# alphacep/vosk-tts

Measured on AMD Instinct MI355X. Metric: audio_samples_per_sec, higher is better.
Workload: dtype f32

## Files before the change

vosk_tts_amd/csrc/engine_model.hip.h:

```cpp
#pragma once
struct ConvW {
  float* w = nullptr;
  float* w16 = nullptr;
  float* wb = nullptr;
  float* bias = nullptr;
  int M = 0, Mpad = 0, Cin = 0, K = 0, n_sg = 0;
};
struct EncLayerW {
  ConvW qkv, o, f1, f2;
  float *ek = nullptr, *ev = nullptr, *g1 = nullptr, *b1 = nullptr, *g2 = nullptr, *b2 = nullptr;
};
struct EncoderW {
  std::vector<EncLayerW> layers;
  int H = 0, F = 0, K = 0;
  int nh = 0, W = 0;
};
struct DDSW {
  std::vector<float*> sw, sb, g1, b1, g2, b2;
  std::vector<float*> swk[3];
  std::vector<float*> wt;
  std::vector<ConvW> pw;
};
struct ConvFlowW {
  float *pre_w = nullptr, *pre_b = nullptr;
  DDSW dds;
  ConvW proj;
};
struct CouplingW {
  ConvW pre, post;
  EncoderW enc;
  std::vector<ConvW> in_layers, rs_layers;
  std::vector<ConvW> rsx;
  ConvW skip_post;
  int cond_off = 0;
};
struct MonoW {
  EncoderW enc;
  float *post_w = nullptr, *post_b = nullptr;
};
struct ResBlockW {
  ConvW c1[VITS_MAX_RESD], c2[VITS_MAX_RESD];
  int K = 0;
  int dil[VITS_MAX_RESD] = {0};
};
struct UpW {
  ConvW w;
  int u = 0, Ku = 0, cout = 0, taps = 0, pad_l = 0, halo = 0;
  int shift[8] = {0};
};
struct DecNeeds {
  int pre_out = 0, post_out = 0, tail_cols = 0;
  int ups_q[VITS_MAX_UPS] = {0};
  int c1_out[VITS_MAX_UPS][VITS_MAX_RESD] = {{0}}, c2_out[VITS_MAX_UPS][VITS_MAX_RESD] = {{0}};
};
struct DecGeom {
  struct Stage {
    int cin = 0, cout = 0;
    int u = 0, taps = 0;
    int rate_in = 1, rate_out = 1;
  } st[VITS_MAX_UPS];
  int n_ups = 0;
  int post_rows = 1, post_pad = 3;
  bool reflect = false;
  bool has_mb = false;
  int final_rate = 1;
  long long samples_per_frame = 1;
  DecNeeds needs;
  int rag_halo = 32;
};
static DecGeom dec_geom(const vits_hparams& hp) {
  DecGeom G;
  const bool istft = hp.dec_type == 0 || hp.dec_type == 2 || hp.dec_type == 3, filt = hp.dec_type == 0 || hp.dec_type == 2;
  G.n_ups = hp.n_ups;
  double rf = 3.0;
  double span = 0;
  for (int j = 0; j < hp.n_resk; ++j) {
    double sp = 0;
    for (int d = 0; d < hp.n_resd; ++d) sp += (hp.res_kernels[j] - 1) * hp.res_dilations[j][d] / 2.0 + (hp.res_kernels[j] - 1) / 2.0;
    if (sp > span) span = sp;
  }
  long long rate = 1;
  int C = hp.dec_initial_channel;
  for (int i = 0; i < hp.n_ups; ++i) {
    DecGeom::Stage& S = G.st[i];
    S.u = hp.up_rates[i]; S.taps = (hp.up_kernels[i] + S.u - 1) / S.u;
    S.cin = C; S.cout = C / 2;
    S.rate_in = (int)rate;
    rf += (double)(S.taps / 2 + 1) / (double)rate;
    rate *= S.u;
    S.rate_out = (int)rate;
    rf += span / (double)rate;
    C = S.cout;
  }
  G.final_rate = (int)rate;
  G.samples_per_frame = istft ? rate * hp.istft_hop * hp.subbands : rate;
  G.reflect = istft; G.post_pad = istft ? 4 : 3;
  G.post_rows = istft ? hp.subbands * (hp.istft_n_fft + 2) : 1;
  G.has_mb = filt;
  rf += 4.0 / (double)rate;
  if (filt) rf += ((double)hp.istft_n_fft / hp.istft_hop + (hp.pqmf_taps / 2.0) / hp.subbands / hp.istft_hop) / (double)rate;
  if (hp.dec_type == 3) rf += ((double)hp.istft_n_fft / hp.istft_hop) / (double)rate;
  G.rag_halo = std::max((int)ceil(rf) + 2, 32);

  DecNeeds& N = G.needs;
  int need = 0;
  if (istft) need = (hp.istft_n_fft + hp.istft_hop - 1) / hp.istft_hop + 2;
  if (filt) need += ((hp.pqmf_taps / 2 + hp.subbands - 1) / hp.subbands + hp.istft_hop - 1) / hp.istft_hop;
  N.tail_cols = need;
  N.post_out = need + 1;
  need += 4;
  for (int i = hp.n_ups - 1; i >= 0; --i) {
    for (int d = hp.n_resd - 1; d >= 0; --d) {
      int h2 = 0, h1 = 0;
      for (int j = 0; j < hp.n_resk; ++j) {
        const int k = hp.res_kernels[j];
        h2 = std::max(h2, (k - 1) / 2);
// ... 69 lines not shown

static const float* tget(vits_model* m, int ndim, int d0, int d1, int d2, const char* fmt, ...) {
  char name[160];
  va_list ap;
  va_start(ap, fmt);
  vsnprintf(name, sizeof name, fmt, ap);
  va_end(ap);
  for (uint32_t i = 0; i < m->n_entries; ++i) {
    const vits_blob_entry* e = &m->entries[i];
    if (strncmp(e->name, name, sizeof e->name) == 0) {
      const int want[3] = {d0, d1, d2};
      if ((int)e->ndim != ndim) { m->missing = true; fail(VITS_ERR_BLOB, "tensor %s: ndim %u != %d", name, e->ndim, ndim); return nullptr; }
      for (int k = 0; k < ndim && k < 3; ++k)
        if (want[k] >= 0 && (int)e->dims[k] != want[k]) {
          m->missing = true;
          fail(VITS_ERR_BLOB, "tensor %s: dim %d is %u, expected %d", name, k, e->dims[k], want[k]);
          return nullptr;
        }
      return reinterpret_cast<const float*>(m->blob + e->offset);
    }
  }
  m->missing = true;
  fail(VITS_ERR_BLOB, "tensor %s missing from blob", name);
  return nullptr;
}

static bool thas(const vits_model* m, const char* name) {
  for (uint32_t i = 0; i < m->n_entries; ++i)
    if (strncmp(m->entries[i].name, name, sizeof m->entries[i].name) == 0) return true;
  return false;
}

static size_t align_up(size_t v, size_t a) { return (v + a - 1) / a * a; }

static void* weight_alloc(vits_model* m, size_t bytes) {
  bytes = align_up(bytes ? bytes : 4, 256);
  constexpr size_t guard = (size_t)64 << 10;
  if (m->slab_used + bytes + guard > m->slab_bytes) {
    size_t want = m->blob_bytes + m->blob_bytes / 4 + ((size_t)8 << 20);
    if (!m->allocs.empty()) want = (size_t)32 << 20;
    if (want < bytes + guard) want = bytes + guard;
    want = align_up(want, (size_t)2 << 20);
    void* d = nullptr;
    if (hipMalloc(&d, want) != hipSuccess) return nullptr;
    m->allocs.push_back(d);
    m->slab = static_cast<char*>(d);
    m->slab_bytes = want;
    m->slab_used = 0;
  }
  void* p = m->slab + m->slab_used;
  m->slab_used += bytes;
  return p;
}

static float* upload(vits_model* m, const float* host, size_t n) {
  if (!host) return nullptr;
  void* d = weight_alloc(m, n * sizeof(float));
  if (!d) { m->missing = true; fail(VITS_ERR_NOMEM, "hipMalloc of %zu floats failed", n); return nullptr; }
  if (hipMemcpy(d, host, n * sizeof(float), hipMemcpyHostToDevice) != hipSuccess) { m->missing = true; fail(VITS_ERR_DEVICE, "hipMemcpy H2D failed"); return nullptr; }
  return static_cast<float*>(d);
}

template <typename F, typename F16>
static ConvW make_conv2(vits_model* m, int M, int Cin, int K, const float* bias, F src, bool small16, F16 src16) {
  ConvW c;
  c.M = M; c.Mpad = cdiv(M, 32) * 32; c.Cin = Cin; c.K = K;
  if (Cin % CONV_CI_T != 0) { m->missing = true; fail(VITS_ERR_UNSUPPORTED, "conv C_in=%d is not a multiple of %d", Cin, CONV_CI_T); return c; }
  c.n_sg = Cin / CONV_CI_T * 2 * K;
  std::vector<float> packed((size_t)c.Mpad * Cin * K);
  pack_conv_weights(packed.data(), c.Mpad, Cin, K, [&](int row, int ci, int kk) -> float { return row < M ? src(row, ci, kk) : 0.f; });
  c.w = upload(m, packed.data(), packed.size());
  if (small16) {
    const int Mp16 = cdiv(M, 16) * 16;
    packed.assign((size_t)Mp16 * Cin * K, 0.f);
    pack_conv_weights16(packed.data(), Mp16, Cin, K, [&](int row, int ci, int kk) -> float { return row < M ? src16(row, ci, kk) : 0.f; });
    c.w16 = upload(m, packed.data(), packed.size());
  }
  c.bias = bias ? upload(m, bias, M) : nullptr;
  return c;
}
template <typename F>
static ConvW make_conv(vits_model* m, int M, int Cin, int K, const float* bias, F src, bool small16 = true) {
  return make_conv2(m, M, Cin, K, bias, src, small16, src);
}

template <typename F>
static void add_bf3_packing(vits_model* m, ConvW& c, F src) {
  if (!c.w || c.Mpad % 32 || c.Cin % CONV_CI_T) return;
  std::vector<uint16_t> pk((size_t)c.Mpad * c.Cin * c.K * 2 + 2 * 128 * 8, 0);
  const int M = c.M;
  pack_conv_weights_bf3(pk.data(), c.Mpad, c.Cin, c.K, [&](int row, int ci, int kk) -> float { return row < M ? src(row, ci, kk) : 0.f; });
  c.wb = upload(m, reinterpret_cast<const float*>(pk.data()), pk.size() / 2);
}
static ConvW conv_from(vits_model* m, const char* name, int Cout, int Cin, int K, bool has_bias, bool small16 = true, bool bf3 = false) {
  const float* w = tget(m, 3, Cout, Cin, K, "%s.weight", name);
  const float* b = has_bias ? tget(m, 1, Cout, -1, -1, "%s.bias", name) : nullptr;
  if (m->missing) return ConvW();
  auto src = [&](int r, int ci, int kk) { return w[((size_t)r * Cin + ci) * K + kk]; };
  ConvW c = make_conv(m, Cout, Cin, K, b, src, small16);
  if (bf3) add_bf3_packing(m, c, src);
  return c;
}

static void load_encoder(vits_model* m, EncoderW& E, const char* pfx, int n_layers, int H, int F, int K, int nh, int W) {
  const vits_hparams& hp = m->hp;
  const int dk = H / nh, NW = 2 * W + 1;
  E.H = H; E.F = F; E.K = K; E.nh = nh; E.W = W;
  E.layers.resize(n_layers);
  char nm[200];
  for (int i = 0; i < n_layers && !m->missing; ++i) {
    EncLayerW& L = E.layers[i];
    const float* wq = tget(m, 3, H, H, 1, "%s.attn_layers.%d.conv_q.weight", pfx, i);
    const float* wk = tget(m, 3, H, H, 1, "%s.attn_layers.%d.conv_k.weight", pfx, i);
    const float* wv = tget(m, 3, H, H, 1, "%s.attn_layers.%d.conv_v.weight", pfx, i);
    const float* bq = tget(m, 1, H, -1, -1, "%s.attn_layers.%d.conv_q.bias", pfx, i);
    const float* bk = tget(m, 1, H, -1, -1, "%s.attn_layers.%d.conv_k.bias", pfx, i);
    const float* bv = tget(m, 1, H, -1, -1, "%s.attn_layers.%d.conv_v.bias", pfx, i);
    if (m->missing) return;
    std::vector<float> b3(3 * H);
    memcpy(b3.data(), bq, sizeof(float) * H); memcpy(b3.data() + H, bk, sizeof(float) * H); memcpy(b3.data() + 2 * H, bv, sizeof(float) * H);
    auto qkv_src = [&](int r, int ci, int) {
      const float* w = r < H ? wq : (r < 2 * H ? wk : wv);
      return w[(size_t)(r % H) * H + ci];
    };
    L.qkv = make_conv(m, 3 * H, H, 1, b3.data(), qkv_src);
    const bool bf3 = hp.conv_precision == 1 && H % 64 == 0 && F % 64 == 0;
    if (bf3) add_bf3_packing(m, L.qkv, qkv_src);
    snprintf(nm, sizeof nm, "%s.attn_layers.%d.conv_o", pfx, i);
    L.o = conv_from(m, nm, H, H, 1, true, true, bf3);
    if (W >= 0) {
      L.ek = upload(m, tget(m, 3, 1, NW, dk, "%s.attn_layers.%d.emb_rel_k", pfx, i), (size_t)NW * dk);
      L.ev = upload(m, tget(m, 3, 1, NW, dk, "%s.attn_layers.%d.emb_rel_v", pfx, i), (size_t)NW * dk);
    }
    snprintf(nm, sizeof nm, "%s.ffn_layers.%d.conv_1", pfx, i);
    L.f1 = conv_from(m, nm, F, H, K, true, true, bf3);
    snprintf(nm, sizeof nm, "%s.ffn_layers.%d.conv_2", pfx, i);
    L.f2 = conv_from(m, nm, H, F, K, true, true, bf3);
    L.g1 = upload(m, tget(m, 1, H, -1, -1, "%s.norm_layers_1.%d.gamma", pfx, i), H);
    L.b1 = upload(m, tget(m, 1, H, -1, -1, "%s.norm_layers_1.%d.beta", pfx, i), H);
    L.g2 = upload(m, tget(m, 1, H, -1, -1, "%s.norm_layers_2.%d.gamma", pfx, i), H);
    L.b2 = upload(m, tget(m, 1, H, -1, -1, "%s.norm_layers_2.%d.beta", pfx, i), H);
  }
}

static void load_dds(vits_model* m, DDSW& D, const char* pfx, int C, int K, int n) {
  char nm[200];
  for (int i = 0; i < n && !m->missing; ++i) {
    D.sw.push_back(upload(m, tget(m, 3, C, 1, K, "%s.convs_sep.%d.weight", pfx, i), (size_t)C * K));
    if (K == 3 && !m->missing) {
      const float* w = tget(m, 3, C, 1, K, "%s.convs_sep.%d.weight", pfx, i);
      for (int k = 0; k < 3; ++k) {
        std::vector<float> t(C);
        for (int c = 0; c < C; ++c) t[c] = w[(size_t)c * 3 + k];
        D.swk[k].push_back(upload(m, t.data(), t.size()));
      }
    }
    D.sb.push_back(upload(m, tget(m, 1, C, -1, -1, "%s.convs_sep.%d.bias", pfx, i), C));
    snprintf(nm, sizeof nm, "%s.convs_1x1.%d", pfx, i);
    D.pw.push_back(conv_from(m, nm, C, C, 1, true));
    {
      const float* w = tget(m, 3, C, C, 1, "%s.weight", nm);
      std::vector<float> t((size_t)C * C);
      if (w && C % 4 == 0) for (int co = 0; co < C; ++co) for (int ci = 0; ci < C; ++ci) t[((size_t)(ci / 4) * C + co) * 4 + (ci & 3)] = w[(size_t)co * C + ci];
      D.wt.push_back(upload(m, t.data(), t.size()));
    }
    D.g1.push_back(upload(m, tget(m, 1, C, -1, -1, "%s.norms_1.%d.gamma", pfx, i), C));
// ... 234 lines not shown
      snprintf(nm, sizeof nm, "dp.flows.%d.convs", 2 * k + 1);
      load_dds(m, c.dds, nm, D, hp.dp_kernel_size, hp.dp_dds_layers);
      snprintf(nm, sizeof nm, "dp.flows.%d.proj", 2 * k + 1);
      c.proj = conv_from(m, nm, P, D, 1, true);
    }
    {
      const float* em = tget(m, 2, 2, 1, -1, "dp.flows.0.m");
      const float* el = tget(m, 2, 2, 1, -1, "dp.flows.0.logs");
      if (m->missing) return VITS_ERR_BLOB;
      m->ea_m = upload(m, em, 2); m->ea_logs = upload(m, el, 2);
    }
  }

  m->flow.resize(hp.flow_n_flows);
  if (mono) m->mono.resize(hp.flow_n_flows);
  const int K5 = hp.flow_kernel_size, L = hp.flow_wn_layers;
  for (int f = 0; f < hp.flow_n_flows && !m->missing; ++f) {
    CouplingW& c = m->flow[f];
    const int fi = (mono ? 3 : 2) * f;
    snprintf(nm, sizeof nm, "flow.flows.%d.pre", fi);
    c.pre = conv_from(m, nm, H, I / 2, 1, true);
    snprintf(nm, sizeof nm, "flow.flows.%d.pre_transformer", fi);
    if (hp.flow_type == 0) load_encoder(m, c.enc, nm, 1, H, H, K5, 2, hp.window_size);
    else if (hp.flow_type == 1) load_encoder(m, c.enc, nm, 2, I / 2, I / 2, 3, 2, -1);
    for (int i = 0; i < L && !m->missing; ++i) {
      const float* w = tget(m, 3, 2 * H, H, K5, "flow.flows.%d.enc.in_layers.%d.weight", fi, i);
      const float* b = tget(m, 1, 2 * H, -1, -1, "flow.flows.%d.enc.in_layers.%d.bias", fi, i);
      if (m->missing) break;
      auto gate_src = [&](int r, int ci, int kk) {
        const int j = r / 64, q = r % 64;
        const int orig = q < 32 ? j * 32 + q : H + j * 32 + (q - 32);
        return w[((size_t)orig * H + ci) * K5 + kk];
      };
      c.in_layers.push_back(make_conv2(m, 2 * H, H, K5, b, gate_src, true, [&](int r, int ci, int kk) {
        const int j = r / 16, q = r % 16;
        const int orig = q < 8 ? j * 8 + q : H + j * 8 + (q - 8);
        return w[((size_t)orig * H + ci) * K5 + kk];
      }));
      if (hp.conv_precision == 1 && (2 * H) % 128 == 0) add_bf3_packing(m, c.in_layers.back(), gate_src);
      snprintf(nm, sizeof nm, "flow.flows.%d.enc.res_skip_layers.%d", fi, i);
      c.rs_layers.push_back(conv_from(m, nm, i < L - 1 ? 2 * H : H, H, 1, true));
    }
    if (m->use_g)
      c.cond_off = add_cond(tget(m, 3, 2 * H * L, G, 1, "flow.flows.%d.enc.cond_layer.weight", fi),
                            tget(m, 1, 2 * H * L, -1, -1, "flow.flows.%d.enc.cond_layer.bias", fi), 2 * H * L);
    snprintf(nm, sizeof nm, "flow.flows.%d.post", fi);
    c.post = conv_from(m, nm, I / 2, H, 1, true);
    if (!m->missing) {
      const float* pw = tget(m, 3, I / 2, H, 1, "%s.weight", nm);
      const float* pb = tget(m, 1, I / 2, -1, -1, "%s.bias", nm);
      std::vector<const float*> rw(L), rb(L);
      for (int i = 0; i < L; ++i) {
        const int rows = i < L - 1 ? 2 * H : H;
        rw[i] = tget(m, 3, rows, H, 1, "flow.flows.%d.enc.res_skip_layers.%d.weight", fi, i);
        rb[i] = tget(m, 1, rows, -1, -1, "flow.flows.%d.enc.res_skip_layers.%d.bias", fi, i);
      }
      if (!m->missing) {
        for (int i = 0; i < L - 1; ++i) {
          auto rs_src = [&](int r, int ci, int) { return rw[i][(size_t)r * H + ci]; };
          c.rsx.push_back(make_conv(m, H, H, 1, rb[i], rs_src));
          if (hp.conv_precision == 1 && H % 64 == 0) add_bf3_packing(m, c.rsx.back(), rs_src);
        }
        const int half = I / 2;
        std::vector<double> Wf((size_t)half * L * H, 0.0), bf(half, 0.0);
        for (int o = 0; o < half; ++o) {
          double bacc = pb[o];
          for (int i = 0; i < L; ++i) {
            const int off = i < L - 1 ? H : 0;
            for (int k = 0; k < H; ++k) {
              const double pwk = pw[(size_t)o * H + k];
              bacc += pwk * rb[i][off + k];
              const float* wr = rw[i] + (size_t)(off + k) * H;
              double* dst = &Wf[((size_t)o * L + i) * H];
              for (int ci = 0; ci < H; ++ci) dst[ci] += pwk * wr[ci];
            }
          }
          bf[o] = bacc;
        }
        std::vector<float> bff(half);
        for (int o = 0; o < half; ++o) bff[o] = (float)bf[o];
        c.skip_post = make_conv(m, half, L * H, 1, bff.data(), [&](int r, int ci, int) { return (float)Wf[(size_t)r * L * H + ci]; });
      }
    }
    if (mono && !m->missing) {
      MonoW& mo = m->mono[f];
      const int half = I / 2;
      snprintf(nm, sizeof nm, "flow.flows.%d.pre_transformer", fi + 2);
      load_encoder(m, mo.enc, nm, 2, half, half, 3, 2, -1);
      mo.post_w = upload(m, tget(m, 3, half, half, 1, "flow.flows.%d.post.weight", fi + 2), (size_t)half * half);
      mo.post_b = upload(m, tget(m, 1, half, -1, -1, "flow.flows.%d.post.bias", fi + 2), half);
    }
  }
  if (m->use_g && hp.dec_type == 1)
    m->cond_dec_off = add_cond(tget(m, 3, hp.dec_initial_channel, G, 1, "dec.cond.weight"),
                               tget(m, 1, hp.dec_initial_channel, -1, -1, "dec.cond.bias"), hp.dec_initial_channel);
  if (m->missing) return VITS_ERR_BLOB;
  m->cond_rows = (int)cB.size();
  if (m->cond_rows) { m->cond_W = upload(m, cW.data(), cW.size()); m->cond_b = upload(m, cB.data(), cB.size()); }

  return load_decoder(m);
}
```

vosk_tts_amd/csrc/persist_plan.hip.h:

```cpp
#pragma once

#define PERSIST_SDP 1
#define PERSIST_ENC 2
#define PERSIST_FLOW 4

static int persist_slice(int Cin, int K) {
  if (Cin % 16 || (K != 1 && K != 3 && K != 5)) return 0;
  for (int ks = 1; ks <= 4; ++ks) {
    if (Cin % ks) continue;
    const int cs = Cin / ks;
    if (cs % 16 == 0 && cs <= PS_MAXC && (cs / 16) * K <= PS_MAXU * PS_WAVES) return cs;
  }
  return 0;
}
static bool persist_conv_ok(const ConvW& W) { return W.w16 && persist_slice(W.Cin, W.K) > 0; }

static bool persist_encoder_ok(const vits_model* m, const EncoderW& E) {
  (void)m;
  if (E.layers.empty() || E.H % 16 || E.H > PS_MAXC || E.nh < 1 || E.nh > 4 || E.H % E.nh) return false;
  const int dk = E.H / E.nh;
  if (dk > PS_DKP || dk % 16 || E.W < 1 || E.W > 4 || (2 * E.W + 1) * dk > 1024) return false;
  for (const EncLayerW& L : E.layers)
    if (!persist_conv_ok(L.qkv) || !persist_conv_ok(L.o) || !persist_conv_ok(L.f1) || !persist_conv_ok(L.f2) || L.qkv.K != 1 || L.o.K != 1) return false;
  return true;
}

static int persist_max_t() {
  static const int v = getenv("VITS_PS_MAX_T") ? atoi(getenv("VITS_PS_MAX_T")) : PS_MAX_T;
  return v < 16 ? 16 : (v > PS_MAX_T ? PS_MAX_T : v);
}
static bool persist_common_ok(const vits_model* m, int B, int T) {
  return m->acoustic && B == 1 && T >= 1 && T <= persist_max_t() && m->n_cu >= 16 && m->zeros;
}

static bool persist_sdp_eligible(const vits_model* m, int B, int Tx) {
  const vits_hparams& hp = m->hp;
  if (m->dp_det) return false;
  if (!persist_common_ok(m, B, Tx)) return false;
  const int D = hp.dp_filter_channels, H = hp.hidden_channels;
  if (D % 32 || D > PS_MAXC || H % 16 || H > PS_MAXC || hp.dp_kernel_size != 3) return false;
  const int nl = (int)m->dp_dds.pw.size();
  if (nl < 1 || nl > 3 || hp.dp_n_flows < 2 || hp.dp_num_bins > 16 || 3 * hp.dp_num_bins - 1 > 32) return false;
  if (1 + 2 * (nl + 1) * hp.dp_n_flows > PS_MAX_STEPS) return false;
  if (!persist_conv_ok(m->dp_pre) || !persist_conv_ok(m->dp_proj) || (int)m->dp_dds.swk[0].size() != nl) return false;
  for (const ConvW& c : m->dp_dds.pw) if (!persist_conv_ok(c)) return false;
  for (int k = 1; k < hp.dp_n_flows; ++k) {
    if ((int)m->cf[k].dds.pw.size() != nl || (int)m->cf[k].dds.swk[0].size() != nl || !persist_conv_ok(m->cf[k].proj)) return false;
    for (const ConvW& c : m->cf[k].dds.pw) if (!persist_conv_ok(c)) return false;
  }
  return true;
}
static size_t persist_sdp_cells(const vits_model* m, int B, int Tx) {
  if (!persist_sdp_eligible(m, B, Tx)) return 0;
  const vits_hparams& hp = m->hp;
  const size_t Tp = (size_t)cdiv(Tx, 16) * 16, D = hp.dp_filter_channels, nl = m->dp_dds.pw.size(), nf = hp.dp_n_flows;
  return Tp * (D * (1 + nf * (3 * nl + 2)) + 2 * (nf + 1));
}

static size_t persist_enc_layer_cells(const vits_model* m, const EncoderW& E, size_t Tp) {
  const size_t H = E.H, F = E.F, nh = E.nh, dk = H / nh, ntn = Tp / 16;
  const size_t ks2 = E.layers[0].f2.Cin / persist_slice(E.layers[0].f2.Cin, E.layers[0].f2.K);
  return Tp * (3 * H + ntn * nh * (dk + 2) + H + H + H + F + ks2 * H + H);
}
static bool persist_enc_eligible(const vits_model* m, int B, int Tx) {
  const vits_hparams& hp = m->hp;
  if (!persist_common_ok(m, B, Tx) || !persist_encoder_ok(m, m->enc_p) || !persist_conv_ok(m->enc_proj) || m->enc_proj.K != 1) return false;
  if (hp.bert_dim > 0 && (!persist_conv_ok(m->bert_proj) || m->bert_proj.K != 1)) return false;
  return 4 + 8 * (int)m->enc_p.layers.size() <= PS_MAX_STEPS;
}
static size_t persist_enc_cells(const vits_model* m, int B, int Tx) {
  if (!persist_enc_eligible(m, B, Tx)) return 0;
  const size_t Tp = (size_t)cdiv(Tx, 16) * 16, H = m->hp.hidden_channels;
  size_t bert = 0;
  if (m->hp.bert_dim > 0) bert = Tp * H * (m->bert_proj.Cin / persist_slice(m->bert_proj.Cin, 1) + 1);
  return Tp * H + bert + m->enc_p.layers.size() * persist_enc_layer_cells(m, m->enc_p, Tp);
}

static bool persist_flow_eligible(const vits_model* m, int B, int Ty) {
  const vits_hparams& hp = m->hp;
  if (hp.flow_type != 0) return false;
  if (!persist_common_ok(m, B, Ty) || hp.flow_n_flows < 1) return false;
  const int I = hp.inter_channels, H = hp.hidden_channels, L = hp.flow_wn_layers;
  if (I % 32 || I > PS_MAXC || L < 1 || L > 4 || H % 16 || H > PS_MAXC || (I / 2) % 16) return false;
  for (const CouplingW& C : m->flow) {
    if (!persist_conv_ok(C.pre) || C.pre.K != 1 || !persist_encoder_ok(m, C.enc) || C.enc.layers.size() != 1) return false;
    if ((int)C.in_layers.size() != L || (int)C.rsx.size() != L - 1 || !C.skip_post.w16 || C.skip_post.Cin != L * H) return false;
    for (const ConvW& c : C.in_layers) if (!persist_conv_ok(c) || persist_slice(c.Cin, c.K) != c.Cin) return false;
    for (const ConvW& c : C.rsx) if (!persist_conv_ok(c) || c.K != 1) return false;
  }
  return hp.flow_n_flows * (11 + 2 * L) <= PS_MAX_STEPS;
}
static size_t persist_flow_cells(const vits_model* m, int B, int Ty) {
  if (!persist_flow_eligible(m, B, Ty)) return 0;
  const vits_hparams& hp = m->hp;
  const size_t Tp = (size_t)cdiv(Ty, 16) * 16, H = hp.hidden_channels, I = hp.inter_channels, L = hp.flow_wn_layers;
  const size_t per = Tp * (H + L * H + (L - 1) * H + L * (I / 2) + I) + persist_enc_layer_cells(m, m->flow[0].enc, Tp);
  return per * hp.flow_n_flows;
}

enum { PS_EPI_STORE = 0, PS_EPI_SPLINE = 1, PS_EPI_GATE = 2 };
struct PStep {
  int kind;
  int Tp;
  int Cin;
  int cin_pitch;
  int c_off, c_sign;
  int Cout, n_mb;
  int G, mbg, ks;
  int K, pad;
  int epi, relu;
  int in_mask, out_mask;
  int ypitch, y_off;
  int gate_H;
  int plain_T;
  int zinit;
  int blen;
  const float* w16;
  const float* bias;
  const float* cond;
  const ll_t* bin;
  const float* bin_plain;
  const ll_t* res;
  int rpitch;
  ll_t* yout;
  float* yplain;
  const ll_t* z;
  ll_t* zout;
  int z_row;
  int last, ea_row;
  int C, plen;
  int padd[8];
  const float* par[8];
  const float* vec;
  int dil, dw, fin;
  const ll_t* xin; const ll_t* y2;
  ll_t* xout;
  ll_t* bout;
  int np, ln;
  const ll_t* part; long long part_stride;
  const ll_t* base;
  const float* emb; float scale; int n_vocab;
  int nh, dk, W;
  const ll_t* qkv;
  ll_t* ap;
  const float* ek; const float* ev;
  const ll_t* u; const float* u_plain;
  int H;
  ll_t* out;
  float* oplain;
};

static const float* persist_pack(vits_session* s, const float* const (&src)[8], const int (&add)[8], int len, int rows) {
  vits_model* m = s->m;
  std::vector<long long> key;
  for (int k = 0; k < 8; ++k) { key.push_back((long long)(uintptr_t)src[k]); key.push_back(add[k]); }
  key.push_back(len); key.push_back(rows);
  for (auto& pk : s->ps_pending)
    if (pk.first == key) return pk.second;
  float* dst = nullptr;
  {
    std::lock_guard<std::mutex> g(m->pack_mu);
    auto it = m->packs.find(key);
    if (it != m->packs.end()) return it->second;
    if (hipMalloc((void**)&dst, sizeof(float) * 8 * (size_t)rows) != hipSuccess) return nullptr;
    m->allocs.push_back(dst);
  }
  PsPackArgs a;
  for (int k = 0; k < 8; ++k) { a.src[k] = src[k] == m->zeros ? nullptr : src[k]; a.add[k] = add[k]; a.len[k] = len; }
  hipLaunchKernelGGL(ps_pack_kernel, dim3(cdiv(rows * 8, 256)), dim3(256), 0, s->stream, dst, a, rows);
  s->ps_pending.emplace_back(std::move(key), dst);
  return dst;
}
static void persist_publish_packs(vits_session* s, bool ok) {
  if (ok && !s->ps_pending.empty()) {
    std::lock_guard<std::mutex> g(s->m->pack_mu);
    for (auto& pk : s->ps_pending) s->m->packs.emplace(pk.first, pk.second);
  }
  s->ps_pending.clear();
}

struct PBuild {
  vits_model* m;
  std::vector<PStep>* steps;
  ll_t* cur;
  ll_t* end;
  int T, Tp, ntn;
  double flops = 0;
  bool overflow = false;
  ll_t* take(size_t cells) {
    ll_t* p = cur;
    cur += cells;
    if (cur > end) overflow = true;
    return p;
  }
  ll_t* take_rows(size_t ch) { return take(ch * (size_t)Tp); }
  PStep blank(int kind) const {
    PStep st;
    memset(&st, 0, sizeof st);
    st.kind = kind;
    st.Cin = 16; st.cin_pitch = 16; st.c_sign = 1; st.Cout = 16; st.n_mb = 1; st.G = 1; st.mbg = 1; st.ks = 1; st.K = 1; st.blen = 16;
    st.C = 16; st.plen = 256; st.plain_T = T; st.np = 0; st.nh = 1; st.dk = 16;
    st.w16 = st.bias = st.cond = m->zeros;
    for (int k = 0; k < 8; ++k) st.par[k] = m->zeros;
    return st;
  }
  PStep& push(const PStep& st) {
    if ((int)steps->size() >= PS_MAX_STEPS) { overflow = true; return steps->back(); }
    steps->push_back(st);
    steps->back().Tp = Tp;
    return steps->back();
  }
  PStep mm(const ConvW& W, const ll_t* bin, int cin_pitch, int c_off = 0, int c_sign = 1) {
    PStep st = blank(PK_MM);
    const int cs = persist_slice(W.Cin, W.K);
    st.Cin = cs; st.ks = W.Cin / cs; st.cin_pitch = cin_pitch; st.c_off = c_off; st.c_sign = c_sign;
    st.K = W.K; st.pad = (W.K - 1) / 2;
    st.Cout = W.M; st.n_mb = cdiv(W.M, 16); st.blen = W.M;
    st.w16 = W.w16;
    st.bias = (st.ks == 1 && W.bias) ? W.bias : m->zeros;
    st.bin = bin;
    st.ypitch = cdiv(W.M, 16) * 16;
    set_groups(st);
    flops += 2.0 * T * (double)W.M * W.Cin * W.K;
    return st;
  }
  void set_groups(PStep& st) const {
    st.mbg = cdiv(st.n_mb * ntn * st.ks, m->n_cu);
    st.G = cdiv(st.n_mb, st.mbg);
    while (ntn * st.G * st.ks > m->n_cu && st.mbg < st.n_mb) { ++st.mbg; st.G = cdiv(st.n_mb, st.mbg); }
  }
  void col_par(PStep& st, int C, const float* p0, const float* p1, const float* p2, const float* vec) {
    st.C = C; st.plen = C;
    st.par[0] = p0 ? p0 : m->zeros; st.par[1] = p1 ? p1 : m->zeros; st.par[2] = p2 ? p2 : m->zeros;
    st.vec = vec;
  }
};

static const ll_t* persist_encoder_layer(PBuild& b, const EncLayerW& L, const EncoderW& E, const ll_t* x, const float* vec_next, const ll_t* base,
                                         float* xplain) {
  vits_model* m = b.m;
  const int H = E.H, F = E.F, nh = E.nh, dk = H / nh, W = E.W, Tp = b.Tp, ntn = b.ntn;
  PStep st = b.mm(L.qkv, x, H);
  st.yout = b.take_rows(3 * H);
  const ll_t* qkv = b.push(st).yout;
  st = b.blank(PK_ATT);
  st.nh = nh; st.dk = dk; st.W = W; st.qkv = qkv;
  st.ap = b.take((size_t)ntn * Tp * nh * (dk + 2));
  if (W > 0 && L.ek && L.ev) { st.ek = L.ek; st.ev = L.ev; }
  else st.W = 0;
  b.flops += 4.0 * (double)H * b.T * b.T;
  const ll_t* ap = b.push(st).ap;
  st = b.blank(PK_MERGE);
  st.C = H; st.nh = nh; st.dk = dk; st.ap = const_cast<ll_t*>(ap);
  st.out = b.take_rows(H);
  const ll_t* att = b.push(st).out;
  st = b.mm(L.o, att, H);
  st.res = x; st.rpitch = H;
  st.yout = b.take_rows(H);
  const ll_t* y1 = b.push(st).yout;
  st = b.blank(PK_LN);
  b.col_par(st, H, L.g1, L.b1, nullptr, nullptr);
  st.np = 1; st.ln = 1; st.part = y1; st.part_stride = 0;
  st.out = b.take_rows(H);
  const ll_t* x1 = b.push(st).out;
  st = b.mm(L.f1, x1, H);
  st.in_mask = 1; st.relu = 1; st.out_mask = 1;
  st.yout = b.take_rows(F);
  const ll_t* hcell = b.push(st).yout;
  st = b.mm(L.f2, hcell, cdiv(F, 16) * 16);
  st.in_mask = 1;
  const int ks = st.ks;
  st.yout = b.take_rows((size_t)ks * H);
  st.ypitch = H;
  const ll_t* part = b.push(st).yout;
  st = b.blank(PK_LN);
  b.col_par(st, H, L.g2, L.b2, ks > 1 ? L.f2.bias : nullptr, vec_next);
  st.np = ks; st.ln = 1; st.part = part; st.part_stride = (long long)Tp * H; st.res = x1;
  st.base = base;
  st.out = b.take_rows(H);
  st.oplain = xplain;
  return b.push(st).out;
}

static void persist_resolve(vits_session* s, const std::vector<PStep>& steps, int P, int seg_pstep, int& seg_step, std::vector<PRec>& recs, bool& bad) {
  vits_model* m = s->m;
  int Tp = 16, ntn = 1;
  seg_step = -1;
  auto U = [](const void* p) { return (unsigned long long)(uintptr_t)p; };
  PRec idle;
  memset(&idle, 0, sizeof idle);
  idle.kf = PK_IDLE; idle.a1 = 16;
  for (int k = 6; k < 10; ++k) idle.p[k] = U(m->zeros);
  recs.clear();
  auto new_step = [&]() -> PRec* { recs.insert(recs.end(), (size_t)P, idle); return recs.data() + recs.size() - P; };
  std::vector<int> rank_of, used;
  auto place = [&](int Q) {
    const int items = Q * ntn;
    rank_of.assign(items, -1);
    if (P % 8 || P / 8 < ntn) { for (int i = 0; i < items; ++i) rank_of[i] = i; return; }
    used.assign(P, 0);
    const int per = P / 8, cap = per / ntn;
    for (int q = 0; q < Q && q < 8 * cap; ++q)
      for (int j = 0; j < ntn; ++j) {
        const int rk = (q % 8) + 8 * ((q / 8) * ntn + j);
        rank_of[q * ntn + j] = rk;
        used[rk] = 1;
      }
    int nx = 0;
    for (int i = 8 * cap * ntn; i < items; ++i) {
      while (used[nx]) ++nx;
      rank_of[i] = nx;
      used[nx] = 1;
    }
  };
  for (size_t si = 0; si < steps.size(); ++si) {
    const PStep& st = steps[si];
    Tp = st.Tp; ntn = Tp / 16;
    if ((int)si == seg_pstep) seg_step = (int)(recs.size() / P);
    if (st.kind == PK_DUR) {
      PRec* R = new_step();
      PRec& r = R[0];
      r.kf = PK_DUR | (st.dw ? 0 : PF_PLAIN_IN);
      r.a1 = st.C; r.a2 = st.dil;
      r.p[0] = U(s->ps_x_logw); r.p[1] = U(s->dur); r.p[2] = U(s->cum); r.p[3] = U(s->ps_x_cum);
      r.p[4] = U(s->len_y); r.p[5] = U(s->ylen64); r.p[6] = U(s->ps_x_leny);
    } else if (st.kind == PK_EXPAND) {
      PRec* R = nullptr;
      for (int t = 0; t < Tp; ++t) {
        if (t % P == 0) R = new_step();
        PRec& r = R[t % P];
        r.kf = PK_EXPAND | (st.dw ? 0 : PF_PLAIN_IN);
        r.a1 = st.C; r.a2 = t; r.a3 = s->Tx;
        r.p[0] = st.dw ? U(s->ps_x_stats) : U(s->stats);
        r.p[1] = st.dw ? U(s->ps_x_cum) : U(s->cum);
        r.p[3] = U(st.out); r.p[4] = U(st.oplain);
        r.b[4] = st.plain_T;
      }
    } else if (st.kind == PK_MM) {
      const int items = ntn * st.G * st.ks;
      if (items > P) { bad = true; return; }
      PRec* R = new_step();
      const int n_u = st.Cin / 16 * st.K;
      const bool gate = st.epi == PS_EPI_GATE;
      if (n_u > 127 || st.mbg > 15) { bad = true; return; }
      place(st.G * st.ks);
      for (int item = 0; item < items; ++item) {
        const int j = item % ntn, q = item / ntn, g = q % st.G, slice = q / st.G;
        const int n0 = j * 16, mb0 = g * st.mbg, nblk = std::min(st.mbg, st.n_mb - mb0);
        PRec& r = R[rank_of[q * ntn + j]];
        r.kf = PK_MM | (st.relu ? PF_RELU : 0) | (st.in_mask ? PF_INMASK : 0) | (st.out_mask ? PF_OUTMASK : 0) | (gate ? PF_GATE : 0) |
               (st.epi == PS_EPI_SPLINE ? PF_SPLINE : 0) | ((st.zinit && g == 0 && slice == 0) ? PF_ZINIT : 0) | (st.last ? PF_LAST : 0) |
               (st.bin_plain ? PF_PLAIN_IN : 0);
        r.a1 = st.Cin | (st.K << 16);
        r.a2 = st.bin_plain ? st.c_sign : st.cin_pitch * st.c_sign;
        r.a3 = n0 - st.pad;
        const int ch0 = st.c_off + st.c_sign * slice * st.Cin;
        if (st.bin_plain) r.p[0] = U(st.bin_plain + (size_t)ch0 * st.plain_T);
        else r.p[0] = U(st.bin + (st.c_sign > 0 ? ch0 : ch0 - (st.Cin - 1)));
        const int row0 = gate ? mb0 * 8 : mb0 * 16;
        r.p[1] = st.yout ? U(st.yout + ((size_t)slice * Tp + n0) * st.ypitch + st.y_off + row0) : 0;
        r.p[2] = st.yplain ? U(st.yplain + (size_t)row0 * st.plain_T + n0) : 0;
        r.p[3] = st.res ? U(st.res + (size_t)n0 * st.rpitch + row0) : 0;
        r.p[4] = U(st.z); r.p[5] = U(st.zout);
        r.p[6] = U(st.w16 + ((size_t)mb0 * st.ks + slice) * n_u * 256);
        r.p[7] = U(st.bias + (st.bias == m->zeros ? 0 : row0));
        r.p[8] = U(st.cond + (st.cond == m->zeros ? 0 : row0));
        r.b[0] = n_u | (nblk << 7);
        r.b[1] = st.ks * n_u * 256;
        r.b[2] = st.ypitch;
        r.b[3] = gate ? 2 * st.gate_H : st.Cout - row0;
        r.b[4] = st.plain_T; r.b[5] = st.rpitch;
        r.b[6] = n0 | (st.z_row << 16) | (st.ea_row << 20);
        r.b[7] = st.gate_H;
      }
    } else if (st.kind == PK_ATT) {
      const int items = st.nh * ntn * ntn;
      const int add[8] = {0, 512, 0, 512, 0, 0, 0, 0};
      const float* const src[8] = {st.ek, st.ek, st.ev, st.ev, nullptr, nullptr, nullptr, nullptr};
      const float* pack = m->zeros;
      if (st.W > 0) {
        const float* const sk[8] = {st.ek, st.ek, st.ev, st.ev, m->zeros, m->zeros, m->zeros, m->zeros};
        (void)src;
        pack = persist_pack(s, sk, add, (2 * st.W + 1) * st.dk, 512);
        if (!pack) { bad = true; return; }
      }
      for (int i0 = 0; i0 < items; i0 += P) {
        PRec* R = new_step();
        for (int item = i0; item < std::min(items, i0 + P); ++item) {
          const int kt = item % ntn, qt = (item / ntn) % ntn, hd = item / (ntn * ntn);
          PRec& r = R[item - i0];
          r.kf = PK_ATT;
          r.a1 = st.dk | (st.nh << 8) | (st.W << 16);
          r.a2 = (qt * 16) | ((kt * 16) << 16);
          r.a3 = hd | (kt << 8);
          r.p[0] = U(st.qkv); r.p[1] = U(st.ap); r.p[9] = U(pack);
        }
      }
    } else {
      PRec* R = nullptr;
      const float* pack = m->zeros;
      if (st.kind != PK_MERGE && st.kind != PK_EMB) {
        pack = persist_pack(s, st.par, st.padd, st.plen, 256);
        if (!pack) { bad = true; return; }
      }
      for (int t = 0; t < Tp; ++t) {
        if (t % P == 0) R = new_step();
        PRec& r = R[t % P];
        r.a1 = st.C; r.a2 = t; r.p[9] = U(pack);
        r.p[3] = U(st.out); r.p[4] = U(st.oplain);
        r.b[4] = st.plain_T;
        if (st.kind == PK_DDS) {
          r.kf = PK_DDS | (st.dw ? PF_DW : 0) | (st.fin == 1 ? PF_FIN_LN : 0) | (st.fin == 2 ? PF_FIN_PRE : 0);
          r.a1 = st.C | (st.dil << 16);
          r.p[0] = U(st.xin); r.p[1] = U(st.y2); r.p[2] = st.z ? U(st.z + (size_t)st.z_row * Tp) : 0; r.p[3] = U(st.xout); r.p[4] = U(st.bout);
        } else if (st.kind == PK_LN) {
          r.kf = PK_LN | (st.ln ? PF_LN : 0);
          r.a3 = st.np;
          r.p[0] = U(st.part); r.p[1] = U(st.res); r.p[2] = U(st.base);
          r.p[8] = U(st.vec ? st.vec : m->zeros);
          r.b[0] = (int)(unsigned)(st.part_stride & 0xffffffffll); r.b[1] = (int)(st.part_stride >> 32);
        } else if (st.kind == PK_EMB) {
          r.kf = PK_EMB;
          r.p[0] = U(st.emb);
          r.p[8] = U(st.vec ? st.vec : m->zeros);
          memcpy(&r.b[0], &st.scale, 4);
          r.b[1] = st.n_vocab;
        } else if (st.kind == PK_MERGE) {
          r.kf = PK_MERGE;
          r.a3 = st.dk | (st.nh << 8);
          r.p[0] = U(st.ap);
          r.b[0] = Tp * st.nh * (st.dk + 2);
        } else {
          r.kf = PK_COUPLE | (st.u_plain ? PF_PLAIN_IN : 0);
          r.a3 = st.np | (st.H << 16);
          r.p[0] = U(st.part); r.p[1] = U(st.u); r.p[2] = U(st.u_plain);
          r.b[0] = (int)(unsigned)(st.part_stride & 0xffffffffll); r.b[1] = (int)(st.part_stride >> 32);
        }
      }
    }
    if ((int)(recs.size() / P) > PS_MAX_STEPS) { bad = true; return; }
  }
}

static void persist_upload(vits_session* s, vits_session::PersistProg& pp, PBuild& b) {
  pp.flops = b.flops;
  pp.ok = false;
  if (b.overflow) return;
  vits_model* m = s->m;
  const int P = m->n_cu;
  std::vector<PRec> recs;
  bool bad = false;
  int seg_step = -1;
  persist_resolve(s, *b.steps, P, pp.h.seg_step, seg_step, recs, bad);
  if (bad || recs.empty() || (pp.h.seg_step >= 0 && seg_step < 0)) return;
  pp.h.seg_step = seg_step;
  const size_t bytes = recs.size() * sizeof(PRec);
  if (bytes > pp.recs_bytes) {
    if (pp.recs_d) { hipStreamSynchronize(s->stream); hipFree(pp.recs_d); pp.recs_d = nullptr; pp.recs_bytes = 0; }
    if (hipMalloc((void**)&pp.recs_d, bytes) != hipSuccess) { pp.recs_d = nullptr; return; }
    pp.recs_bytes = bytes;
  }
  if (!pp.d && hipMalloc((void**)&pp.d, sizeof(PProgram)) != hipSuccess) { pp.d = nullptr; return; }
  pp.h.n_steps = (int)(recs.size() / P);
  pp.h.P = P;
  pp.h.recs = pp.recs_d;
  pp.kinds.clear();
  for (int i = 0; i < pp.h.n_steps; ++i) {
    int k = 0;
    for (int w = 0; w < P && !k; ++w) k = recs[(size_t)i * P + w].kf & 0xff;
    pp.kinds.push_back(k);
  }
  pp.recs_h.swap(recs);
  if (hipMemcpyAsync(pp.recs_d, pp.recs_h.data(), bytes, hipMemcpyHostToDevice, s->stream) != hipSuccess) return;
  if (hipMemcpyAsync(pp.d, &pp.h, sizeof(PProgram), hipMemcpyHostToDevice, s->stream) != hipSuccess) return;
  pp.ok = true;
}
static void seg_geom(PBuild& b, int T) { b.T = T; b.Tp = cdiv(T, 16) * 16; b.ntn = b.Tp / 16; }
static void seg_cells(PBuild& b, vits_session::PersistProg& region) { b.cur = region.ll; b.end = region.ll + region.cells; }

static void persist_begin(vits_session* s, vits_session::PersistProg& pp, PBuild& b, std::vector<PStep>& steps, int T, const int* len) {
  vits_model* m = s->m;
  memset(&pp.h, 0, sizeof(PProgram));
  steps.clear();
  steps.reserve(PS_MAX_STEPS + 1);
  b.m = m; b.steps = &steps; b.cur = pp.ll; b.end = pp.ll + pp.cells;
  seg_geom(b, T);
  PProgram& P = pp.h;
  P.T = T; P.Tp = b.Tp;
  P.nb = m->hp.dp_num_bins; P.bound = m->hp.dp_tail_bound; P.inv_sqrt_d = 1.0f / sqrtf((float)m->hp.dp_filter_channels);
  P.len = len; P.ea_m = m->ea_m ? m->ea_m : m->zeros; P.ea_logs = m->ea_logs ? m->ea_logs : m->zeros; P.logw = s->logw; P.err = s->d_err;
  P.seg_step = -1;
}

static const ll_t* seg_enc(vits_session* s, PBuild& b, ll_t* stats_cells) {
  vits_model* m = s->m;
  const vits_hparams& hp = m->hp;
  const int H = hp.hidden_channels, n = (int)m->enc_p.layers.size();
  const int cond_layer = (m->use_g && m->cond_enc_off >= 0) ? hp.enc_cond_layer : -1;
  const float* vec = cond_layer >= 0 ? s->condv + m->cond_enc_off : nullptr;
  const bool bert = hp.bert_dim > 0;
  PStep st = b.blank(PK_EMB);
  b.col_par(st, H, nullptr, nullptr, nullptr, (cond_layer == 0 && !bert) ? vec : nullptr);
  st.emb = m->emb; st.scale = sqrtf((float)H); st.n_vocab = hp.n_vocab;
  st.out = b.take_rows(H);
  const ll_t* x = b.push(st).out;
  if (bert) {
    st = b.mm(m->bert_proj, nullptr, hp.bert_dim);
    st.bin_plain = s->ps_bert;
    const int ks = st.ks;
    st.yout = b.take_rows((size_t)ks * H);
    st.ypitch = H;
    const ll_t* part = b.push(st).yout;
    st = b.blank(PK_LN);
    b.col_par(st, H, nullptr, nullptr, ks > 1 ? m->bert_proj.bias : nullptr, cond_layer == 0 ? vec : nullptr);
    st.np = ks; st.ln = 0; st.part = part; st.part_stride = (long long)b.Tp * H; st.res = x;
    st.out = b.take_rows(H);
    x = b.push(st).out;
  }
  for (int i = 0; i < n; ++i)
    x = persist_encoder_layer(b, m->enc_p.layers[i], m->enc_p, x, (i + 1 == cond_layer) ? vec : nullptr, nullptr, i == n - 1 ? s->x : nullptr);
  st = b.mm(m->enc_proj, x, H);
  st.in_mask = 1; st.out_mask = 1;
  st.yplain = s->stats;
  st.yout = stats_cells;
  b.push(st);
  return x;
}

static void seg_sdp(vits_session* s, PBuild& b, const ll_t* x_cells) {
  vits_model* m = s->m;
  const vits_hparams& hp = m->hp;
  std::vector<PStep>& steps = *b.steps;
  const int D = hp.dp_filter_channels, nl = (int)m->dp_dds.pw.size(), K = hp.dp_kernel_size, H = hp.hidden_channels;
  PStep st = b.mm(m->dp_pre, x_cells, H);
  if (!x_cells) st.bin_plain = s->x;
  if (m->use_g && m->cond_dp_off >= 0) st.cond = s->condv + m->cond_dp_off;
  st.zinit = 1;
  st.yout = b.take_rows(D); st.zout = b.take_rows(2);
  const size_t first = steps.size();
  const ll_t* x = b.push(st).yout;
  const ll_t* z = steps[first].zout;
  auto stack = [&](const DDSW& Wd, const ConvW& proj, bool spline, const ll_t* xin, const ll_t* zc, int z_row, const float* pw, const float* pb) -> PStep& {
    const ll_t* y2 = nullptr;
    int dil = 1;
    for (int i = 0; i <= nl; ++i) {
      const bool fin = i == nl;
      st = b.blank(PK_DDS);
      st.C = D; st.plen = D; st.dw = fin ? 0 : 1; st.dil = fin ? 0 : dil;
      st.xin = xin; st.y2 = y2;
      if (i > 0) { st.fin = 1; st.par[0] = Wd.g2[i - 1]; st.par[1] = Wd.b2[i - 1]; }
      else if (zc) { st.fin = 2; st.z = zc; st.z_row = z_row; st.par[0] = pw; st.par[1] = pb; }
      if (!fin) {
        st.par[2] = Wd.sb[i]; st.par[3] = Wd.swk[0][i]; st.par[4] = Wd.swk[1][i]; st.par[5] = Wd.swk[2][i];
        st.par[6] = Wd.g1[i]; st.par[7] = Wd.b1[i];
        st.bout = b.take_rows(D);
      }
      st.xout = b.take_rows(D);
      b.flops += 2.0 * b.T * (double)D * (fin ? 0 : K);
      const PStep& col = b.push(st);
      xin = col.xout;
      st = b.mm(fin ? proj : Wd.pw[i], fin ? col.xout : col.bout, D);
      if (fin) {
        if (spline) { st.epi = PS_EPI_SPLINE; st.mbg = st.n_mb; st.G = 1; }
        else st.out_mask = 1;
        return b.push(st);
      }
      st.yout = b.take_rows(D);
      y2 = b.push(st).yout;
      dil *= K;
    }
    return steps[first];
  };
  {
    PStep& pj = stack(m->dp_dds, m->dp_proj, false, x, nullptr, 0, nullptr, nullptr);
    pj.yout = b.take_rows(D);
  }
  const ll_t* dc = steps.back().yout;
  int swap = 0;
  for (int k = hp.dp_n_flows - 1; k >= 1; --k) {
    swap ^= 1;
    const ConvFlowW& c = m->cf[k];
    PStep& pj = stack(c.dds, c.proj, true, dc, z, swap, c.pre_w, c.pre_b);
    pj.z = z; pj.z_row = swap;
    if (k > 1) { pj.zout = b.take_rows(2); z = pj.zout; }
    else { pj.last = 1; pj.ea_row = swap ^ 1; }
  }
}

static void seg_flow(vits_session* s, PBuild& b, const ll_t* zp_cells) {
  vits_model* m = s->m;
  const vits_hparams& hp = m->hp;
  const int H = hp.hidden_channels, I = hp.inter_channels, half = I / 2, L = hp.flow_wn_layers;
  const ll_t* u = zp_cells;
  for (int f = hp.flow_n_flows - 1; f >= 0; --f) {
    const CouplingW& C = m->flow[f];
    PStep st = b.mm(C.pre, u, I, I - 1, -1);
    if (!u) st.bin_plain = s->zA;
    st.out_mask = 1;
    st.yout = b.take_rows(H);
    const ll_t* fh = b.push(st).yout;
    const ll_t* fx = persist_encoder_layer(b, C.enc.layers[0], C.enc, fh, nullptr, fh, nullptr);
    ll_t* acts = b.take_rows((size_t)L * H);
    for (int i = 0; i < L; ++i) {
      st = b.mm(C.in_layers[i], fx, H);
      st.in_mask = 1; st.epi = PS_EPI_GATE; st.gate_H = H; st.blen = 2 * H;
      st.n_mb = cdiv(2 * H, 16); st.Cout = 2 * H;
      b.set_groups(st);
      if (m->use_g) st.cond = s->condv + C.cond_off + i * 2 * H;
      st.yout = acts; st.ypitch = L * H; st.y_off = i * H;
      b.push(st);
      if (i == L - 1) break;
      st = b.mm(C.rsx[i], acts, L * H, i * H, 1);
      st.res = fx; st.rpitch = H; st.out_mask = 1;
      st.yout = b.take_rows(H);
      fx = b.push(st).yout;
    }
    st = b.mm(C.skip_post, acts, L * H);
    const int ks = st.ks;
    st.yout = b.take_rows((size_t)ks * half); st.ypitch = half;
    const ll_t* part = b.push(st).yout;
    st = b.blank(PK_COUPLE);
    b.col_par(st, I, nullptr, nullptr, ks > 1 ? C.skip_post.bias : nullptr, nullptr);
    st.plen = half; st.padd[2] = -half;
    st.H = half; st.np = ks; st.part = part; st.part_stride = (long long)b.Tp * half;
    st.u = u; st.u_plain = u ? nullptr : s->zA;
    st.out = b.take_rows(I);
    if (f == 0) st.oplain = s->zB;
    u = b.push(st).out;
  }
}

static void seg_dur(vits_session* s, PBuild& b, bool with_logw, int Tcap) {
  PStep st = b.blank(PK_DUR);
  st.C = s->Tx; st.dil = Tcap; st.dw = with_logw ? 1 : 0;
  b.push(st);
}
static const ll_t* seg_expand(vits_session* s, PBuild& b, bool cells) {
  PStep st = b.blank(PK_EXPAND);
  st.C = s->m->hp.inter_channels; st.dw = cells ? 1 : 0;
  st.out = s->ps_x_zp;
  st.oplain = s->zA;
  return b.push(st).out;
}

static void persist_build_enc(vits_session* s) {
  vits_session::PersistProg& pp = s->ps_enc;
  PBuild b;
  std::vector<PStep> steps;
  persist_begin(s, pp, b, steps, s->Tx, s->len_x);
  seg_enc(s, b, nullptr);
  persist_upload(s, pp, b);
}
static void persist_build_sdp(vits_session* s) {
  vits_session::PersistProg& pp = s->ps_sdp;
  PBuild b;
  std::vector<PStep> steps;
  persist_begin(s, pp, b, steps, s->Tx, s->len_x);
  seg_sdp(s, b, nullptr);
  persist_upload(s, pp, b);
}
static void persist_build_flow(vits_session* s) {
  vits_session::PersistProg& pp = s->ps_flow;
  PBuild b;
  std::vector<PStep> steps;
  persist_begin(s, pp, b, steps, s->Ty, s->len_y);
  seg_flow(s, b, nullptr);
  persist_upload(s, pp, b);
}

static void persist_build_front(vits_session* s, vits_session::PersistProg& pp, bool with_sdp, int Tcap, bool and_back) {
  PBuild b;
  std::vector<PStep> steps;
  persist_begin(s, pp, b, steps, s->Tx, s->len_x);
  pp.h.logw_cells = s->ps_x_logw;
  seg_cells(b, s->ps_enc);
  const ll_t* x = seg_enc(s, b, and_back ? s->ps_x_stats : nullptr);
  if (with_sdp) { seg_cells(b, s->ps_sdp); seg_sdp(s, b, x); }
  seg_dur(s, b, with_sdp, Tcap);
  if (and_back) {
    pp.h.seg_step = (int)steps.size();
    pp.h.T2 = s->Ty; pp.h.Tp2 = cdiv(s->Ty, 16) * 16; pp.h.len2 = s->ps_x_leny;
    seg_geom(b, s->Ty);
    const ll_t* zp = seg_expand(s, b, true);
    seg_cells(b, s->ps_flow);
// ... 57 lines not shown
```

Before: 45.08 million.

## Fold flow pre conv into first-layer QKV and co-schedule independent matmul steps

Precomputes a combined weight that applies the flow coupling's pre projection and the first encoder layer's QKV projection in one matmul, so QKV no longer waits for the pre conv output. The pre conv still runs because its output is the residual base, but it is now marked as joinable and packed into the same persistent-kernel step as the QKV matmul. The same pairing is applied to the SDP pre conv and the preceding matmul. Pairing removes one grid-wide step barrier per pair, at the cost of coarser per-item work (fit_pair raises mbg) so both fit within the CU count, and it adds extra folded weights in memory.

```diff
diff --git a/vosk_tts_amd/csrc/engine_model.hip.h b/vosk_tts_amd/csrc/engine_model.hip.h
--- a/vosk_tts_amd/csrc/engine_model.hip.h
+++ b/vosk_tts_amd/csrc/engine_model.hip.h
@@ -32,6 +32,7 @@
   std::vector<ConvW> in_layers, rs_layers;
   std::vector<ConvW> rsx;
   ConvW skip_post;
+  ConvW qkv_pre;
   int cond_off = 0;
 };
 struct MonoW {
@@ -267,6 +268,18 @@
 template <typename F>
 static ConvW make_conv(vits_model* m, int M, int Cin, int K, const float* bias, F src, bool small16 = true) {
   return make_conv2(m, M, Cin, K, bias, src, small16, src);
+}
+template <typename F>
+static ConvW make_conv16(vits_model* m, int M, int Cin, int K, const float* bias, F src) {
+  ConvW c;
+  c.M = M; c.Mpad = cdiv(M, 32) * 32; c.Cin = Cin; c.K = K;
+  if (Cin % CONV_CI_T != 0) return c;
+  const int Mp16 = cdiv(M, 16) * 16;
+  std::vector<float> packed((size_t)Mp16 * Cin * K, 0.f);
+  pack_conv_weights16(packed.data(), Mp16, Cin, K, [&](int row, int ci, int kk) -> float { return row < M ? src(row, ci, kk) : 0.f; });
+  c.w16 = upload(m, packed.data(), packed.size());
+  c.bias = bias ? upload(m, bias, M) : nullptr;
+  return c;
 }
 
 template <typename F>
@@ -667,6 +680,34 @@
         c.skip_post = make_conv(m, half, L * H, 1, bff.data(), [&](int r, int ci, int) { return (float)Wf[(size_t)r * L * H + ci]; });
       }
     }
+    if (hp.flow_type == 0 && !m->missing && (I / 2) % CONV_CI_T == 0) {
+      const int half = I / 2;
+      const float* pw = tget(m, 3, H, half, 1, "flow.flows.%d.pre.weight", fi);
+      const float* pb = tget(m, 1, H, -1, -1, "flow.flows.%d.pre.bias", fi);
+      const float *aw[3], *ab[3];
+      const char* qkvn[3] = {"q", "k", "v"};
+      for (int j = 0; j < 3; ++j) {
+        aw[j] = tget(m, 3, H, H, 1, "flow.flows.%d.pre_transformer.attn_layers.0.conv_%s.weight", fi, qkvn[j]);
+        ab[j] = tget(m, 1, H, -1, -1, "flow.flows.%d.pre_transformer.attn_layers.0.conv_%s.bias", fi, qkvn[j]);
+      }
+      if (!m->missing) {
+        std::vector<double> Wc((size_t)3 * H * half, 0.0);
+        std::vector<float> bc(3 * H);
+        for (int r = 0; r < 3 * H; ++r) {
+          const float* wr = aw[r / H] + (size_t)(r % H) * H;
+          double bacc = ab[r / H][r % H];
+          double* dst = &Wc[(size_t)r * half];
+          for (int k = 0; k < H; ++k) {
+            const double wk = wr[k];
+            bacc += wk * pb[k];
+            const float* pr = pw + (size_t)k * half;
+            for (int ci = 0; ci < half; ++ci) dst[ci] += wk * pr[ci];
+          }
+          bc[r] = (float)bacc;
+        }
+        c.qkv_pre = make_conv16(m, 3 * H, half, 1, bc.data(), [&](int r, int ci, int) { return (float)Wc[(size_t)r * half + ci]; });
+      }
+    }
     if (mono && !m->missing) {
       MonoW& mo = m->mono[f];
       const int half = I / 2;
diff --git a/vosk_tts_amd/csrc/persist_plan.hip.h b/vosk_tts_amd/csrc/persist_plan.hip.h
--- a/vosk_tts_amd/csrc/persist_plan.hip.h
+++ b/vosk_tts_amd/csrc/persist_plan.hip.h
@@ -102,6 +102,7 @@
 struct PStep {
   int kind;
   int Tp;
+  int join;
   int Cin;
   int cin_pitch;
   int c_off, c_sign;
@@ -229,6 +230,20 @@
     st.G = cdiv(st.n_mb, st.mbg);
     while (ntn * st.G * st.ks > m->n_cu && st.mbg < st.n_mb) { ++st.mbg; st.G = cdiv(st.n_mb, st.mbg); }
   }
+  bool fit_pair(PStep& a, PStep& c) const {
+    const PStep a0 = a, c0 = c;
+    auto work = [](const PStep& st) { return st.mbg * (st.Cin / 16) * st.K; };
+    auto coarser = [](PStep& st) {
+      if (st.epi == PS_EPI_SPLINE || st.mbg >= st.n_mb || st.mbg >= 15) return false;
+      ++st.mbg; st.G = cdiv(st.n_mb, st.mbg);
+      return true;
+    };
+    while (ntn * (a.G * a.ks + c.G * c.ks) > m->n_cu) {
+      const bool c_first = work(c) <= work(a);
+      if (!coarser(c_first ? c : a) && !coarser(c_first ? a : c)) { a = a0; c = c0; return false; }
+    }
+    return true;
+  }
   void col_par(PStep& st, int C, const float* p0, const float* p1, const float* p2, const float* vec) {
     st.C = C; st.plen = C;
     st.par[0] = p0 ? p0 : m->zeros; st.par[1] = p1 ? p1 : m->zeros; st.par[2] = p2 ? p2 : m->zeros;
@@ -237,12 +252,13 @@
 };
 
 static const ll_t* persist_encoder_layer(PBuild& b, const EncLayerW& L, const EncoderW& E, const ll_t* x, const float* vec_next, const ll_t* base,
-                                         float* xplain) {
+                                         float* xplain, const PStep* qkv_st = nullptr, const PStep* joined = nullptr) {
   vits_model* m = b.m;
   const int H = E.H, F = E.F, nh = E.nh, dk = H / nh, W = E.W, Tp = b.Tp, ntn = b.ntn;
-  PStep st = b.mm(L.qkv, x, H);
+  PStep st = qkv_st ? *qkv_st : b.mm(L.qkv, x, H);
   st.yout = b.take_rows(3 * H);
   const ll_t* qkv = b.push(st).yout;
+  if (joined) b.push(*joined);
   st = b.blank(PK_ATT);
   st.nh = nh; st.dk = dk; st.W = W; st.qkv = qkv;
   st.ap = b.take((size_t)ntn * Tp * nh * (dk + 2));
@@ -313,6 +329,43 @@
       used[nx] = 1;
     }
   };
+  auto mm_items = [&](const PStep& st) { return (st.Tp / 16) * st.G * st.ks; };
+  auto emit_mm = [&](const PStep& st, PRec* R, int q0) -> bool {
+    const int items = ntn * st.G * st.ks;
+    const int n_u = st.Cin / 16 * st.K;
+    const bool gate = st.epi == PS_EPI_GATE;
+    if (n_u > 127 || st.mbg > 15) return false;
+    for (int item = 0; item < items; ++item) {
+      const int j = item % ntn, q = item / ntn, g = q % st.G, slice = q / st.G;
+      const int n0 = j * 16, mb0 = g * st.mbg, nblk = std::min(st.mbg, st.n_mb - mb0);
+      PRec& r = R[rank_of[(q0 + q) * ntn + j]];
+      r.kf = PK_MM | (st.relu ? PF_RELU : 0) | (st.in_mask ? PF_INMASK : 0) | (st.out_mask ? PF_OUTMASK : 0) | (gate ? PF_GATE : 0) |
+             (st.epi == PS_EPI_SPLINE ? PF_SPLINE : 0) | ((st.zinit && g == 0 && slice == 0) ? PF_ZINIT : 0) | (st.last ? PF_LAST : 0) |
+             (st.bin_plain ? PF_PLAIN_IN : 0);
+      r.a1 = st.Cin | (st.K << 16);
+      r.a2 = st.bin_plain ? st.c_sign : st.cin_pitch * st.c_sign;
+      r.a3 = n0 - st.pad;
+      const int ch0 = st.c_off + st.c_sign * slice * st.Cin;
+      if (st.bin_plain) r.p[0] = U(st.bin_plain + (size_t)ch0 * st.plain_T);
+      else r.p[0] = U(st.bin + (st.c_sign > 0 ? ch0 : ch0 - (st.Cin - 1)));
+      const int row0 = gate ? mb0 * 8 : mb0 * 16;
+      r.p[1] = st.yout ? U(st.yout + ((size_t)slice * Tp + n0) * st.ypitch + st.y_off + row0) : 0;
+      r.p[2] = st.yplain ? U(st.yplain + (size_t)row0 * st.plain_T + n0) : 0;
+      r.p[3] = st.res ? U(st.res + (size_t)n0 * st.rpitch + row0) : 0;
+      r.p[4] = U(st.z); r.p[5] = U(st.zout);
+      r.p[6] = U(st.w16 + ((size_t)mb0 * st.ks + slice) * n_u * 256);
+      r.p[7] = U(st.bias + (st.bias == m->zeros ? 0 : row0));
+      r.p[8] = U(st.cond + (st.cond == m->zeros ? 0 : row0));
+      r.b[0] = n_u | (nblk << 7);
+      r.b[1] = st.ks * n_u * 256;
+      r.b[2] = st.ypitch;
+      r.b[3] = gate ? 2 * st.gate_H : st.Cout - row0;
+      r.b[4] = st.plain_T; r.b[5] = st.rpitch;
+      r.b[6] = n0 | (st.z_row << 16) | (st.ea_row << 20);
+      r.b[7] = st.gate_H;
+    }
+    return true;
+  };
   for (size_t si = 0; si < steps.size(); ++si) {
     const PStep& st = steps[si];
     Tp = st.Tp; ntn = Tp / 16;
@@ -337,42 +390,13 @@
         r.b[4] = st.plain_T;
       }
     } else if (st.kind == PK_MM) {
-      const int items = ntn * st.G * st.ks;
-      if (items > P) { bad = true; return; }
+      const PStep* nx = si + 1 < steps.size() ? &steps[si + 1] : nullptr;
+      if (nx && !(nx->kind == PK_MM && nx->join && nx->Tp == st.Tp && (int)si + 1 != seg_pstep && mm_items(st) + mm_items(*nx) <= P)) nx = nullptr;
+      if (mm_items(st) > P) { bad = true; return; }
       PRec* R = new_step();
-      const int n_u = st.Cin / 16 * st.K;
-      const bool gate = st.epi == PS_EPI_GATE;
-      if (n_u > 127 || st.mbg > 15) { bad = true; return; }
-      place(st.G * st.ks);
-      for (int item = 0; item < items; ++item) {
-        const int j = item % ntn, q = item / ntn, g = q % st.G, slice = q / st.G;
-        const int n0 = j * 16, mb0 = g * st.mbg, nblk = std::min(st.mbg, st.n_mb - mb0);
-        PRec& r = R[rank_of[q * ntn + j]];
-        r.kf = PK_MM | (st.relu ? PF_RELU : 0) | (st.in_mask ? PF_INMASK : 0) | (st.out_mask ? PF_OUTMASK : 0) | (gate ? PF_GATE : 0) |
-               (st.epi == PS_EPI_SPLINE ? PF_SPLINE : 0) | ((st.zinit && g == 0 && slice == 0) ? PF_ZINIT : 0) | (st.last ? PF_LAST : 0) |
-               (st.bin_plain ? PF_PLAIN_IN : 0);
-        r.a1 = st.Cin | (st.K << 16);
-        r.a2 = st.bin_plain ? st.c_sign : st.cin_pitch * st.c_sign;
-        r.a3 = n0 - st.pad;
-        const int ch0 = st.c_off + st.c_sign * slice * st.Cin;
-        if (st.bin_plain) r.p[0] = U(st.bin_plain + (size_t)ch0 * st.plain_T);
-        else r.p[0] = U(st.bin + (st.c_sign > 0 ? ch0 : ch0 - (st.Cin - 1)));
-        const int row0 = gate ? mb0 * 8 : mb0 * 16;
-        r.p[1] = st.yout ? U(st.yout + ((size_t)slice * Tp + n0) * st.ypitch + st.y_off + row0) : 0;
-        r.p[2] = st.yplain ? U(st.yplain + (size_t)row0 * st.plain_T + n0) : 0;
-        r.p[3] = st.res ? U(st.res + (size_t)n0 * st.rpitch + row0) : 0;
-        r.p[4] = U(st.z); r.p[5] = U(st.zout);
-        r.p[6] = U(st.w16 + ((size_t)mb0 * st.ks + slice) * n_u * 256);
-        r.p[7] = U(st.bias + (st.bias == m->zeros ? 0 : row0));
-        r.p[8] = U(st.cond + (st.cond == m->zeros ? 0 : row0));
-        r.b[0] = n_u | (nblk << 7);
-        r.b[1] = st.ks * n_u * 256;
-        r.b[2] = st.ypitch;
-        r.b[3] = gate ? 2 * st.gate_H : st.Cout - row0;
-        r.b[4] = st.plain_T; r.b[5] = st.rpitch;
-        r.b[6] = n0 | (st.z_row << 16) | (st.ea_row << 20);
-        r.b[7] = st.gate_H;
-      }
+      place(st.G * st.ks + (nx ? nx->G * nx->ks : 0));
+      if (!emit_mm(st, R, 0) || (nx && !emit_mm(*nx, R, st.G * st.ks))) { bad = true; return; }
+      if (nx) ++si;
     } else if (st.kind == PK_ATT) {
       const int items = st.nh * ntn * ntn;
       const int add[8] = {0, 512, 0, 512, 0, 0, 0, 0};
@@ -537,6 +561,7 @@
   if (m->use_g && m->cond_dp_off >= 0) st.cond = s->condv + m->cond_dp_off;
   st.zinit = 1;
   st.yout = b.take_rows(D); st.zout = b.take_rows(2);
+  if (x_cells && !steps.empty() && steps.back().kind == PK_MM && steps.back().Tp == b.Tp) { st.join = 1; b.fit_pair(steps.back(), st); }
   const size_t first = steps.size();
   const ll_t* x = b.push(st).yout;
   const ll_t* z = steps[first].zout;
@@ -598,8 +623,17 @@
     if (!u) st.bin_plain = s->zA;
     st.out_mask = 1;
     st.yout = b.take_rows(H);
-    const ll_t* fh = b.push(st).yout;
-    const ll_t* fx = persist_encoder_layer(b, C.enc.layers[0], C.enc, fh, nullptr, fh, nullptr);
+    const ll_t* fx;
+    if (C.qkv_pre.w16 && persist_slice(C.qkv_pre.Cin, 1) == C.qkv_pre.Cin) {
+      PStep q = b.mm(C.qkv_pre, u, I, I - 1, -1);
+      if (!u) q.bin_plain = s->zA;
+      st.join = 1;
+      b.fit_pair(q, st);
+      fx = persist_encoder_layer(b, C.enc.layers[0], C.enc, st.yout, nullptr, st.yout, nullptr, &q, &st);
+    } else {
+      const ll_t* fh = b.push(st).yout;
+      fx = persist_encoder_layer(b, C.enc.layers[0], C.enc, fh, nullptr, fh, nullptr);
+    }
     ll_t* acts = b.take_rows((size_t)L * H);
     for (int i = 0; i < L; ++i) {
       st = b.mm(C.in_layers[i], fx, H);
```

After: 45.89 million, median of 6. 1.8% higher.
